# AlexFuster/Neural_network_image_compression

Measured on AMD Instinct MI355X. Metric: Megapixels/sec encode+decode, higher is better.
Workload: dtype fp32 (split-f16x3 MFMA); 1 GPU; config2: 64x256x256x3 u8 synthetic per GPU, encode+decode (torch seed 1000+rank); global_batch=64, parallelism=dp1, weights=seeded spread init (random-init weights of the architecture)

## Files before the change

neural_network_image_compression_amd/csrc/nic_capi.hip:

```cpp

#include <hip/hip_runtime.h>

#include <algorithm>
#include <atomic>
#include <cmath>
#include <condition_variable>
#include <cstdarg>
#include <cstdio>
#include <cstring>
#include <mutex>
#include <string>
#include <thread>
#include <vector>

#include "../../include/nic.h"
#include "nic_kernels.h"

using namespace nic;

namespace {

thread_local std::string g_err;

int fail(int code, const char* fmt, ...) __attribute__((format(printf, 2, 3)));
// ... 511 lines not shown
    const int64_t want[4] = {L->k, L->k, L->transposed ? L->cout : L->cin, L->transposed ? L->cin : L->cout};
    if (ndim != 4 || shape[0] != want[0] || shape[1] != want[1] || shape[2] != want[2] || shape[3] != want[3])
      return fail(NIC_ESHAPE, "nic_set_weights: %s/kernel expects shape (%lld,%lld,%lld,%lld)", lname.c_str(),
                  (long long)want[0], (long long)want[1], (long long)want[2], (long long)want[3]);
    std::vector<float> packed;
    std::vector<uint16_t> packedx;
    const int kexp = repack_kernel(*L, host, packed, packedx);
    HIP_TRY(hipMemcpy(c->wk[L->id] + m * packed.size(), packed.data(), packed.size() * sizeof(float),
                      hipMemcpyHostToDevice));
    if (!packedx.empty()) {
      HIP_TRY(hipMemcpy(c->wx[L->id] + m * packedx.size(), packedx.data(), packedx.size() * sizeof(uint16_t),
                        hipMemcpyHostToDevice));
      c->wscale[L->id][m] = std::ldexp(1.0f, -kexp);
    }
    if (L->id == L_DCONV8) {
      const std::vector<uint16_t> f = proj_fragments(packed, kexp);
      HIP_TRY(hipMemcpy(c->wproj + m * kProjFrag, f.data(), f.size() * sizeof(uint16_t), hipMemcpyHostToDevice));
    }
    c->have_k[model_id][idx] = true;
  } else if (kind == "bias") {
    if (ndim != 1 || shape[0] != L->cout)
      return fail(NIC_ESHAPE, "nic_set_weights: %s/bias expects shape (%d,)", lname.c_str(), L->cout);
    HIP_TRY(hipMemcpy(c->wb[L->id] + m * L->cout, host, L->cout * sizeof(float), hipMemcpyHostToDevice));
    c->have_b[model_id][idx] = true;
  } else {
    return fail(NIC_EINVAL, "nic_set_weights: '%s' is neither kernel nor bias", kind.c_str());
  }
  return NIC_OK;
}

int nic_weights_ready(nic_ctx* c, int* enc, int* dec) {
  if (!c) return fail(NIC_EINVAL, "nic_weights_ready: NULL ctx");
  if (enc) *enc = models_ready(c, 0);
  if (dec) *dec = models_ready(c, 2);
  return NIC_OK;
}

int nic_latent_shape(int h, int w, int* h8, int* w8) {
  if (h <= 0 || w <= 0) return fail(NIC_ESHAPE, "nic_latent_shape: h=%d w=%d must be positive", h, w);
  const SamePad a = same_pad(same_pad(same_pad(h, 5, 2).out, 5, 2).out, 5, 2);
  const SamePad b = same_pad(same_pad(same_pad(w, 5, 2).out, 5, 2).out, 5, 2);
  if (h8) *h8 = a.out;
  if (w8) *w8 = b.out;
  return NIC_OK;
}

int nic_reserve(nic_ctx* c, int n, int h, int w) {
  if (!c) return fail(NIC_EINVAL, "nic_reserve: NULL ctx");
  if (n < 0 || h <= 0 || w <= 0) return fail(NIC_ESHAPE, "nic_reserve: bad shape (%d,%d,%d)", n, h, w);
  DeviceGuard guard(c->device);
  const EncGeom e = enc_geom(n, h, w);
  const DecGeom d = dec_geom(n, e.c8y.out, e.c8x.out);
  float* R[4];
  int rc = ensure_regions(c, std::max(e.r0, d.r0), std::max(e.r123, d.r123), R);
  if (rc) return rc;
  const size_t cb = n > 0 ? hist_scratch_bytes(n, e.c8y.out * e.c8x.out) : 0;
  if (cb > c->counts_bytes) {
    if (c->counts) HIP_TRY(hipFree(c->counts));
    c->counts = nullptr;
    c->counts_bytes = 0;
    HIP_TRY(hipMalloc(&c->counts, cb));
    c->counts_bytes = cb;
  }
  return NIC_OK;
}

}

namespace {

bool use_k3pair() {
  static const bool on = [] {
    const char* e = getenv("NIC_K3P");
    return !(e && e[0] == '0');
  }();
  return on;
}
hipError_t launch_pair(nic_ctx* c, ConvArgs ap, LayerId lb, hipStream_t st) {
  ap.wx2 = c->wx[lb];
  ap.wscale2[0] = c->wscale[lb][0];
  ap.wscale2[1] = c->wscale[lb][1];
  ap.bias2 = c->wb[lb];
  return launch_k3pair_x3(ap, st);
}

bool use_chain() {
  static const bool on = [] {
    const char* e = getenv("NIC_CHAIN");
    return !(e && e[0] == '0');
  }();
  return on;
}

int encode_pass(nic_ctx* c, const uint8_t* rgb, int n, int h, int w, uint8_t* latent, float* prequant,
                hipStream_t st, bool x3, const RangeGuard& rg, bool timed) {
  const EncGeom g = enc_geom(n, h, w);
  float* R[4];
  int rc = ensure_regions(c, g.r0, g.r123, R);
  if (rc) return rc;
  const int P = 3 * n;
  const bool timing_on = c->timing;
  c->timing = timing_on && timed;
  struct Restore {
    nic_ctx* c;
    bool v;
    ~Restore() { c->timing = v; }
  } restore{c, timing_on};

  Conv1Args a1{};
  a1.rg = rg;
  a1.rgb = rgb;
  a1.out = R[0];
  a1.out_s = x3 ? (uint16_t*)R[0] : nullptr;
  a1.w = c->wk[L_CONV1];
  a1.bias = c->wb[L_CONV1];
  a1.P = P;
  a1.nimg = n;
  a1.H = h;
  a1.W = w;
  a1.OH = g.c1y.out;
  a1.OW = g.c1x.out;
  a1.pad_y = g.c1y.lo;
  a1.pad_x = g.c1x.lo;
  Fp32Chain chain{};
  const bool chained = !x3 && rg.gate && use_chain();
  chain.gate = rg;
  chain.q = c->range + 2;
  const bool fuse12 = x3;
  if (!fuse12) TIMED(L_CONV1, chained ? chain_add_conv1(chain, a1) : launch_conv1(a1, st));
  RangeGuard rgl = rg;
  rgl.trips = nullptr;
  auto run = [&](LayerId id, const ConvArgs& a) {
    return chained ? chain_add_layer(chain, id, a) : x3 ? launch_layer_x3(id, a, st) : launch_layer(id, a, st);
  };

  auto conv = [&](LayerId id, const float* in, float* out, const float* res, int H, int W, int OH, int OW, int py,
                  int px) {
    ConvArgs a{};
    a.rg = rgl;
    a.in = in;
    a.out = out;
    a.res = res;
    a.in_s = (const uint16_t*)in;
    a.out_s = (uint16_t*)out;
    a.res_s = (const uint16_t*)res;
    a.zero16 = c->zero16;
    a.w = c->wk[id];
    a.wx = c->wx[id];
    a.wscale[0] = c->wscale[id][0];
    a.wscale[1] = c->wscale[id][1];
    a.bias = c->wb[id];
    a.P = P;
    a.nimg = n;
    a.H = H;
    a.W = W;
    a.OH = OH;
    a.OW = OW;
    a.pad_y = py;
    a.pad_x = px;
    return a;
  };
  const int h1 = g.c1y.out, w1 = g.c1x.out, h2 = g.c2y.out, w2 = g.c2x.out;
  ConvArgs a2 = conv(L_CONV2, R[0], R[1], nullptr, h1, w1, h2, w2, g.c2y.lo, g.c2x.lo);
  if (fuse12) {
    a2.rgb = rgb;
    a2.wx1 = c->wx[L_CONV1];
// ... 12 lines not shown
  if (x3 && use_k3pair() && k3pair_supported(h2, w2)) {
    TIMED(L_CONV4, launch_pair(c, conv(L_CONV3, R[1], R[3], nullptr, h2, w2, h2, w2, 1, 1), L_CONV4, st));
  } else {
    TIMED(L_CONV3, run(L_CONV3, conv(L_CONV3, R[1], R[2], nullptr, h2, w2, h2, w2, 1, 1)));
    TIMED(L_CONV4, run(L_CONV4, conv(L_CONV4, R[2], R[3], R[1], h2, w2, h2, w2, 1, 1)));
  }
  ConvArgs a8 = conv(L_CONV8, R[3], nullptr, nullptr, h2, w2, g.c8y.out, g.c8x.out, g.c8y.lo, g.c8x.lo);
  a8.out_u8 = latent;
  a8.out_f32_latent = prequant;
  if (x3 && c->fold_part) {
    a8.hist_part = c->fold_part;
  }
  TIMED(L_CONV8, run(L_CONV8, a8));
  if (chained) HIP_TRY(launch_fp32_chain(chain, st));
  return NIC_OK;
}

int decode_pass(nic_ctx* c, const uint8_t* latent, int n, int h8, int w8, uint8_t* rgb, float* rgb_f32,
                hipStream_t st, bool x3, const RangeGuard& rg, bool timed) {
  const DecGeom g = dec_geom(n, h8, w8);
  float* R[4];
  int rc = ensure_regions(c, g.r0, g.r123, R);
  if (rc) return rc;
  const int P = 3 * n;
  const bool timing_on = c->timing;
  c->timing = timing_on && timed;
  struct Restore {
    nic_ctx* c;
    bool v;
    ~Restore() { c->timing = v; }
  } restore{c, timing_on};
  RangeGuard rgl = rg;
  rgl.trips = nullptr;
  Fp32Chain chain{};
  const bool chained = !x3 && rg.gate && use_chain();
  chain.gate = rg;
  chain.q = c->range + 2;
  auto run = [&](LayerId id, const ConvArgs& a) {
    return chained ? chain_add_layer(chain, id, a) : x3 ? launch_layer_x3(id, a, st) : launch_layer(id, a, st);
  };
  auto conv = [&](LayerId id, const float* in, float* out, const float* res, int H, int W, int OH, int OW) {
    ConvArgs a{};
    a.rg = rgl;
    a.in = in;
    a.out = out;
    a.res = res;
    a.in_s = (const uint16_t*)in;
    a.out_s = (uint16_t*)out;
    a.res_s = (const uint16_t*)res;
    a.zero16 = c->zero16;
    a.w = c->wk[id];
    a.wx = c->wx[id];
    a.wscale[0] = c->wscale[id][0];
    a.wscale[1] = c->wscale[id][1];
    a.bias = c->wb[id];
    a.P = P;
    a.nimg = n;
    a.H = H;
    a.W = W;
    a.OH = OH;
    a.OW = OW;
    a.pad_y = 1;
    a.pad_x = 1;
    return a;
  };
  ConvArgs d1 = conv(L_DCONV1, nullptr, R[1], nullptr, h8, w8, 2 * h8, 2 * w8);
  d1.in_u8 = latent;
  d1.rg = rg;
  TIMED(L_DCONV1, run(L_DCONV1, d1));
  const int h2 = 2 * h8, w2 = 2 * w8;
  if (x3 && use_k3pair() && k3pair_supported(h2, w2)) {
    TIMED(L_DCONV6, launch_pair(c, conv(L_DCONV5, R[1], R[3], nullptr, h2, w2, h2, w2), L_DCONV6, st));
  } else {
    TIMED(L_DCONV5, run(L_DCONV5, conv(L_DCONV5, R[1], R[2], nullptr, h2, w2, h2, w2)));
    TIMED(L_DCONV6, run(L_DCONV6, conv(L_DCONV6, R[2], R[3], R[1], h2, w2, h2, w2)));
  }
  ConvArgs d7 = conv(L_DCONV7, R[3], R[0], nullptr, h2, w2, 2 * h2, 2 * w2);
  const bool fuse78 = x3;
  if (fuse78) {
    d7.proj = R[0];
    d7.proj_w = c->wproj;
    d7.proj_scale[0] = c->wscale[L_DCONV8][0];
    d7.proj_scale[1] = c->wscale[L_DCONV8][1];
    TIMED(L_DCONV7, launch_dconv7_proj_x3(d7, st));
  } else {
    TIMED(L_DCONV7, run(L_DCONV7, d7));
  }
  Dconv8Args a8{};
  a8.rg = rgl;
  a8.in = R[0];
  a8.in_s = (const uint16_t*)R[0];
  a8.zero16 = c->zero16;
  a8.out_u8 = rgb;
  a8.out_f32 = rgb_f32;
  a8.w = c->wk[L_DCONV8];
  a8.wx = c->wx[L_DCONV8];
  a8.wscale[0] = c->wscale[L_DCONV8][0];
  a8.wscale[1] = c->wscale[L_DCONV8][1];
  a8.bias = c->wb[L_DCONV8];
  a8.nimg = n;
  a8.H = 2 * h2;
  a8.W = 2 * w2;
  if (fuse78) {
    a8.proj = R[0];
    a8.tiles_y7 = (h2 + 7) / 8;
    a8.tiles_x7 = (w2 + 7) / 8;
    TIMED(L_DCONV8, launch_dconv8_gather(a8, st));
  } else {
    TIMED(L_DCONV8, chained ? chain_add_dconv8(chain, a8) : launch_dconv8(a8, st));
  }
  if (chained) HIP_TRY(launch_fp32_chain(chain, st));
  return NIC_OK;
}

bool x3_plane_fits(long long h64, long long w64) { return h64 * w64 * 64 * 4 < (1LL << 30); }

template <class Pass>
int guarded(nic_ctx* c, hipStream_t st, const char* what, bool x3_fits, Pass pass) {
  if (c->precision != NIC_PRECISION_F16X3 || !x3_fits) return pass(false, RangeGuard{}, true);
  if (++c->epoch <= 0) c->epoch = 1;
  RangeGuard prod{};
  prod.flag = c->range;
  prod.epoch = c->epoch;
  int rc = pass(true, prod, true);
  if (rc) return rc;
  if (c->range_policy == NIC_RANGE_FALLBACK) {
    RangeGuard gate{};
    gate.gate = c->range;
    gate.trips = c->range + 1;
    gate.epoch = c->epoch;
    return pass(false, gate, false);
  }
  HIP_TRY(hipMemcpyAsync(c->range_host, c->range, sizeof(int), hipMemcpyDeviceToHost, st));
  HIP_TRY(hipStreamSynchronize(st));
  if (*c->range_host == c->epoch) {
    ++c->error_trips;
    return fail(NIC_ERANGE, "%s: an activation reached the f16 limit of the split-f16 pass (|x| >= 65504); "
                "outputs are undefined (use NIC_RANGE_FALLBACK or NIC_PRECISION_FP32)", what);
  }
  return NIC_OK;
}

void host_chunk_plan(int n, int k, std::vector<int>& lo) {
  k = std::max(1, std::min({k, n, kHostMaxChunks}));
  std::vector<double> wgt(k);
  double tot = 0;
  for (int i = 0; i < k; ++i)
    tot += wgt[i] = (double)(1 << std::min(i, k - 1 - i));
  lo.assign(1, 0);
  double acc = 0;
  for (int i = 0; i < k; ++i) {
    acc += wgt[i];
    const int b = i + 1 == k ? n : std::max(lo.back() + 1, std::min(n - (k - 1 - i), (int)std::lround(n * acc / tot)));
    lo.push_back(b);
  }
}

bool host_pinned(const void* p) {
  hipPointerAttribute_t a{};
  if (hipPointerGetAttributes(&a, p) != hipSuccess) {
    (void)hipGetLastError();
    return false;
  }
  return a.type == hipMemoryTypeHost;
}

int grow_pinned(uint8_t*& p, size_t& have, size_t need) {
// ... 606 lines not shown
```

neural_network_image_compression_amd/csrc/nic_kernels.h:

```cpp
#pragma once
#include <hip/hip_runtime.h>
#include <stdint.h>

namespace nic {

int set_error(int code, const char* msg);

enum InMode { IN_F32 = 0, IN_U8_LATENT = 1, IN_SPLIT = 2, IN_SPLIT_DMA = 3, IN_U8_CODES = 4 };
enum OutMode { OUT_F32 = 0, OUT_U8_LATENT = 1, OUT_SPLIT = 2 };

enum LayerId {
  L_CONV1 = 0, L_CONV2, L_CONV3, L_CONV4, L_CONV8,
  L_DCONV1, L_DCONV5, L_DCONV6, L_DCONV7, L_DCONV8,
  L_COUNT
};

constexpr float kF16Limit = 65504.0f;
struct RangeGuard {
  int* flag = nullptr;
  const int* gate = nullptr;
  int* trips = nullptr;
  int epoch = 0;
};

// ... 15 lines not shown
  const float* bias;
  int P, nimg;
  int H, W;
  int OH, OW;
  int pad_y, pad_x;
  int tiles_x;
  int tiles_y, ntiles;
  int ws_taps;
  int ws_ngrp;
  int ws_blk[9];
  int ws_xcd;
  uint32_t* hist_part;
  const uint16_t* wx2;
  float wscale2[2];
  const float* bias2;
  int seg_rows;
  const uint8_t* rgb;
  const uint16_t* wx1;
  float wscale1[2];
  const float* bias1;
  int H0, W0;
  int p1y, p1x;
  uint16_t* cplane;
  int cp_h, cp_w;
  float* proj;
  const uint16_t* proj_w;
  float proj_scale[2];
};

struct Conv1Args {
  RangeGuard rg;
  const uint8_t* rgb;
  float* out;
  uint16_t* out_s;
  const float* w;
  const float* bias;
  int P, nimg, H, W, OH, OW, pad_y, pad_x, tiles_x, tiles_y;
};

struct Dconv8Args {
  RangeGuard rg;
  const float* in;
  const uint16_t* in_s;
  const char* zero16;
  uint8_t* out_u8;
  float* out_f32;
  const float* w;
  const uint16_t* wx;
  float wscale[2];
  const float* bias;
  int nimg, H, W, tiles_x, tiles_y;
  const float* proj;
  int tiles_y7, tiles_x7;
};

constexpr int kChainMax = 6;
constexpr int kChainQWords = 2 * kChainMax + 1;
struct Fp32Chain {
  RangeGuard gate;
  int* q;
  int nstage;
  int diag_late;
  int total[kChainMax];
  int kind[kChainMax];
  ConvArgs c[kChainMax];
  Conv1Args c1;
  Dconv8Args d8;
};
hipError_t chain_add_layer(Fp32Chain& ch, LayerId id, ConvArgs a);
hipError_t chain_add_conv1(Fp32Chain& ch, Conv1Args a);
hipError_t chain_add_dconv8(Fp32Chain& ch, Dconv8Args a);
hipError_t launch_fp32_chain(const Fp32Chain& ch, hipStream_t st);
void fp32_chain_launch_info(int* blocks_per_cu, int* grid, int* cooperative);

hipError_t upload_constants(const float* u8_to_unit, const float* ycbcr, const float* ycbcr_inv, const float* off);
hipError_t launch_layer(LayerId id, const ConvArgs& a, hipStream_t st);
hipError_t launch_layer_x3(LayerId id, const ConvArgs& a, hipStream_t st);
bool k3pair_supported(int H, int W);
hipError_t launch_k3pair_x3(const ConvArgs& a, hipStream_t st);
hipError_t launch_conv12_x3(const ConvArgs& a, hipStream_t st);
void c12_plane_geom(int OH, int OW, int pad_y, int pad_x, int p1y, int p1x, int* oy, int* ox, int* hp, int* wp);
hipError_t launch_conv1(Conv1Args a, hipStream_t st);
hipError_t launch_dconv8(Dconv8Args a, hipStream_t st);
hipError_t launch_dconv7_proj_x3(const ConvArgs& a, hipStream_t st);
hipError_t launch_dconv8_gather(Dconv8Args a, hipStream_t st);
size_t hist_scratch_bytes(int nimg, int plane_px);
hipError_t launch_hist(const uint8_t* z, int nimg, int plane_px, uint32_t* part, uint32_t* counts, float* bits,
                       hipStream_t st);
bool hist_fold_supported(int nimg, int h8, int w8);
size_t hist_fold_scratch_bytes(int nimg, int h8, int w8);
hipError_t launch_hist_fold(uint32_t* part, const uint8_t* z, int nimg, int h8, int w8, RangeGuard trip,
                            uint32_t* counts, float* bits, hipStream_t st);
hipError_t launch_pack(const uint8_t* src, uint8_t* dst, int nimg, int h8, int w8, bool unpack, hipStream_t st);

constexpr int kSsimScales = 5;

struct SsimScaleArgs {
  const uint8_t* a8;
  const uint8_t* b8;
  const float* af;
  const float* bf;
  double2* part;
  int P, H, W, tiles_x, tiles;
};

struct SsimCombineArgs {
  const double2* part;
  size_t offset[kSsimScales];
  int tiles[kSsimScales];
  int64_t valid[kSsimScales];
  float* out;
  float* per_scale;
};

struct SsimPlan {
  int h[kSsimScales], w[kSsimScales], tiles_x[kSsimScales], tiles[kSsimScales];
  int64_t valid[kSsimScales];
  size_t img_off[kSsimScales];
  size_t part_off[kSsimScales];
  size_t img_bytes, bytes;
};
hipError_t upload_ssim_constants();
void ssim_plan(int nimg, int H, int W, SsimPlan* plan);
hipError_t launch_ms_ssim(const uint8_t* a, const uint8_t* b, int nimg, int H, int W, void* scratch, float* out,
                          float* per_scale, hipStream_t st);
hipError_t launch_sq_err(const uint8_t* a, const uint8_t* b, int nimg, int64_t bytes, unsigned long long* sse,
                         hipStream_t st);

size_t train_scale_work_floats();
size_t train_wgrad_work_floats(int n, int uh, int uw, int kh, int kw, int ca, int cb);
size_t train_gather_work_bytes(int kh, int kw, int cin, int cout);
hipError_t launch_absmax_scale(const float* x, long long n, float* scale, float* work, hipStream_t st);
hipError_t launch_conv_gather(const float* x, int n, int h, int w, int cin, const float* wt, int kh, int kw, int layout,
                              int stride, int pad_y, int pad_x, int transposed, const float* bias, const float* x_scale,
                              const float* w_scale, float* y, int oh, int ow, int cout, int act, void* work, hipStream_t st);
size_t train_abg_work_floats(long long rows, int cols);
hipError_t launch_act_bias_grad(const float* y, const float* dy, long long rows, int cols, int act, float* dz, float* db,
                                float* dz_scale, float* work, hipStream_t st);
hipError_t launch_conv_wgrad(const float* gat, int n, int gh, int gw, int ca, const float* dir, int uh, int uw, int cb,
                             int kh, int kw, int stride, int pad_y, int pad_x, const float* gat_scale,
                             const float* dir_scale, float* dw, float* work, hipStream_t st);
hipError_t launch_adam_keras(const long long* table, int count, long long max_n, float alpha, float beta1,
                             float beta2, float eps, hipStream_t st);
size_t train_ssim_work_floats(int n, long long hw);
hipError_t launch_ssim_map(const float* mx, const float* my, const float* sxy, const float* sxx, int n, long long hw,
                           float c1, float c2, float* out, float* work, hipStream_t st);
hipError_t launch_ssim_map_grad(const float* mx, const float* my, const float* sxy, const float* sxx, const float* g,
                                int n, long long hw, float c1, float c2, float* gmx, float* gmy, float* gsxy,
                                float* gsxx, hipStream_t st);
hipError_t launch_gauss1d(const float* in, int n, int hi, int wi, const float* taps, int nt, int vertical, int adjoint,
                          float* out, int ho, int wo, hipStream_t st);

}
```

neural_network_image_compression_amd/csrc/nic_kernels.hip:

```cpp

#include <hip/hip_runtime.h>
#include <stdint.h>
#include <stdlib.h>
#include <string.h>

#include <algorithm>
#include <type_traits>
#include <utility>

#include "nic_kernels.h"


namespace nic {

static int device_cus();

typedef float f32x2 __attribute__((ext_vector_type(2)));
typedef float f32x4 __attribute__((ext_vector_type(4)));
template <class F, int... I>
__device__ __forceinline__ void static_for_impl(F&& f, std::integer_sequence<int, I...>) {
  (f(std::integral_constant<int, I>{}), ...);
}
template <int N, class F>
__device__ __forceinline__ void static_for(F&& f) {
// ... 1561 lines not shown
#if defined(NIC_DIAG_C12R) && NIC_DIAG_C12R == 3
      if (false)
#endif
      if (i + 1 < ntile) conv1(i + 1);
      C12R_MARK(3);
      dma_wait_all();
      lds_reads_done();
      C12R_MARK(4);
      stage_barrier();
      C12R_MARK(0);
    }
  }
#ifdef NIC_STAMPS
  if (lane == 0) {
    unsigned long long* o = g_stamps + ((size_t)blockIdx.x * 8 + wave) * 8;
#pragma unroll
    for (int q = 0; q < 7; ++q) o[q] = sx[q];
    o[7] = ntile;
    if (wave == 0) {
      g_stamps[256 * 64 + 2 * blockIdx.x] = __builtin_amdgcn_s_memtime() - s_c0;
      g_stamps[256 * 64 + 2 * blockIdx.x + 1] = __builtin_amdgcn_s_memrealtime() - s_rt0;
    }
  }
#endif
#undef C12R_MARK
  range_report(a.rg, rmax);
}

__device__ __forceinline__ int xcd_pos(int b, int nb) {
  const int x = b & 7, q = nb >> 3, r = nb & 7;
  return x * q + (x < r ? x : r) + (b >> 3);
}

__global__ __launch_bounds__(512) void conv12_kernel(ConvArgs a) {
  KT_SCOPE(1);
  using G = GeomS2<32, 8, 8>;
  __shared__ __attribute__((aligned(16)))
  char lds[2 * G::HALO_BYTES + 4 * 4 * 1024 + 4 * C12_PLANE + 16];
  int gi = 0;
  while (gi + 1 < a.ws_ngrp && (int)blockIdx.x >= a.ws_blk[gi + 1]) ++gi;
  const int nb = a.ws_blk[gi + 1] - a.ws_blk[gi];
  const int bi = xcd_pos(blockIdx.x - a.ws_blk[gi], nb);
  if (__builtin_amdgcn_readfirstlane((int)(threadIdx.x >> 6)) < 4)
    c12r_wave<2>(a, lds, gi, bi, nb);
  else
    c12r_wave<1>(a, lds, gi, bi, nb);
}

template <int CIN, int COUT, int NTS, int TH, int OUT_MODE, bool HIST = false>
__global__ __launch_bounds__(64 * (COUT / 16) * NTS) void conv_ws2_kernel(ConvArgs a) {
  KT_SCOPE(3);
  using G = GeomS2<CIN, TH, 8>;
  constexpr int NCG = COUT / 16;
  static_assert(NCG * NTS == 8, "8 waves per block");
  constexpr int PARTS = 2 * (NTS - 1) * NCG * (TH / 2) * 1024;
  __shared__ __attribute__((aligned(16)))
  char lds[2 * G::HALO_BYTES + PARTS + (HIST ? HIST_LDS : 0)];
  int gi = 0;
  while (gi + 1 < a.ws_ngrp && (int)blockIdx.x >= a.ws_blk[gi + 1]) ++gi;
  const int nb = a.ws_blk[gi + 1] - a.ws_blk[gi];
  const int bi = xcd_pos(blockIdx.x - a.ws_blk[gi], nb);
  const int ts = __builtin_amdgcn_readfirstlane((int)(threadIdx.x >> 6)) / NCG;
  static_for<NTS>([&](auto tsc) {
    constexpr int TS = decltype(tsc)::value;
    if (ts == TS) ws2_wave<CIN, COUT, NTS, TH, OUT_MODE, TS, HIST>(a, lds, gi, bi, nb);
  });
}

template <int CIN, int COUT, int TH, int TW, bool RESID, bool TRP, bool PROJ = false>
__global__ __launch_bounds__(64 * (COUT / 16), 2) void conv_ws_kernel(ConvArgs a) {
  KT_SCOPE(6);
  using G = GeomWS<CIN, TH, TW>;
  __shared__ __attribute__((aligned(16)))
  char lds[2 * G::HALO_BYTES + (PROJ ? 2 * (CIN / 32) * 2 * 64 * 16 + TH * TW * COUT * 4 : 0) +
           (RESID && kResDma ? (COUT / 16) * (TH * TW / 16) * 1024 : 0)];
  const int xcd = blockIdx.x & 7, ng = gridDim.x;
  const int lb = a.ws_xcd ? xcd * (ng >> 3) + min(xcd, ng & 7) + (int)(blockIdx.x >> 3) : (int)blockIdx.x;
  int gi = 0;
  while (gi + 1 < a.ws_ngrp && lb >= a.ws_blk[gi + 1]) ++gi;
  const int bi = lb - a.ws_blk[gi], nb = a.ws_blk[gi + 1] - a.ws_blk[gi];
  const int model = gi & 1;
  if constexpr (!TRP) {
    ws_body<CIN, COUT, TH, TW, RESID, 3, 3, false>(a, lds, model, bi, nb, 0, 0, 0);
  } else if (a.ws_ngrp == 2) {
    ws_body<CIN, COUT, TH, TW, false, 3, 3, true, PROJ>(a, lds, model, bi, nb, 16, 1, 1);
    ws_body<CIN, COUT, TH, TW, false, 2, 3, true, PROJ>(a, lds, model, bi, nb, 4, 0, 1, false);
    ws_body<CIN, COUT, TH, TW, false, 3, 2, true, PROJ>(a, lds, model, bi, nb, 10, 1, 0, false);
    ws_body<CIN, COUT, TH, TW, false, 2, 2, true, PROJ>(a, lds, model, bi, nb, 0, 0, 0, false);
  } else {
    switch (gi >> 1) {
      case 0: ws_body<CIN, COUT, TH, TW, false, 2, 2, true, PROJ>(a, lds, model, bi, nb, 0, 0, 0); break;
      case 1: ws_body<CIN, COUT, TH, TW, false, 2, 3, true, PROJ>(a, lds, model, bi, nb, 4, 0, 1); break;
      case 2: ws_body<CIN, COUT, TH, TW, false, 3, 2, true, PROJ>(a, lds, model, bi, nb, 10, 1, 0); break;
      default: ws_body<CIN, COUT, TH, TW, false, 3, 3, true, PROJ>(a, lds, model, bi, nb, 16, 1, 1); break;
    }
  }
}

constexpr int D1_PSB = 64;
constexpr int D1_RPB = 800;
constexpr int D1_HB = 10 * D1_RPB;
constexpr int D1A_LD = 2;
#ifndef NIC_D1A_PF
#define NIC_D1A_PF 2
#endif

template <int KH1, int KW1, int TB1, int PY1, int PX1, int KH2, int KW2, int TB2, int PY2, int PX2>
__device__ __forceinline__ void d1all_wave(const ConvArgs& a, char* lds, int model, int bi, int nb) {
  constexpr int COUT = 64, MT = 4, TAP_BYTES = 32 * COUT * 4, PXB = COUT * 4;
  constexpr int NT1 = KH1 * KW1, NT2 = KH2 * KW2;
  const int wave = __builtin_amdgcn_readfirstlane(threadIdx.x >> 6), cg = wave & 3;
  const int lane = threadIdx.x & 63, g = lane >> 4, l16 = lane & 15;
  const int per_plane = a.tiles_y * a.tiles_x;
  const int p0 = model ? a.nimg : 0, np = model ? a.P - a.nimg : a.nimg;
  const int ntot = np * per_plane;
  const int ntile = bi < ntot ? (ntot - bi + nb - 1) / nb : 0;
  if (ntile == 0) return;

  f16x8 w1[NT1][2], w2[NT2][2];
  float scale;
  f32x4 bias;
  auto load_weights = [&](int m) __attribute__((always_inline)) {
    const char* wsrc = (const char*)a.wx + (size_t)m * 25 * TAP_BYTES;
    auto frag_w = [&](int tap, int hl) {
      return *(const f16x8*)(wsrc + (size_t)tap * TAP_BYTES + ((((g >> 1) * 2 + hl) * 2 + (g & 1)) * COUT + cg * 16 + l16) * 16);
    };
#pragma unroll
    for (int t = 0; t < NT1; ++t)
#pragma unroll
      for (int hl = 0; hl < 2; ++hl) w1[t][hl] = frag_w(TB1 + t, hl);
#pragma unroll
    for (int t = 0; t < NT2; ++t)
#pragma unroll
      for (int hl = 0; hl < 2; ++hl) w2[t][hl] = frag_w(TB2 + t, hl);
    scale = a.wscale[m] * 0.0039215688593685627f;
    bias = *(const f32x4*)(a.bias + m * COUT + cg * 16 + 4 * g);
  };
  load_weights(model);

  int st_lds[D1A_LD], st_hy[D1A_LD], st_hx[D1A_LD];
#pragma unroll
  for (int j = 0; j < D1A_LD; ++j) {
    const int q = threadIdx.x + 512 * j, pix = q >> 3;
    st_hy[j] = q < 800 ? pix / 10 : -1000;
    st_hx[j] = pix - (pix / 10) * 10;
    st_lds[j] = (pix / 10) * D1_RPB + st_hx[j] * D1_PSB + (q & 7) * 8;
  }
  uint32_t cqa[D1A_LD], cqb[D1A_LD];
  TileWalk it_ld, it_run;
  it_ld.init(bi, nb, a.tiles_y, a.tiles_x);
  it_run = it_ld;
  const size_t img_bytes = (size_t)a.H * a.W * 96;
  auto load_codes = [&](uint32_t (&cq)[D1A_LD], bool live) __attribute__((always_inline)) {
    int pl, ty, tx;
    it_ld.take(pl, ty, tx);
    const int p = p0 + pl, type = p / a.nimg;
    const __amdgpu_buffer_rsrc_t rs = __builtin_amdgcn_make_buffer_rsrc(
        (void*)(a.in_u8 + (live ? (size_t)(p % a.nimg) * img_bytes + type * 32 : 0)), (short)0,
        live ? (int)(img_bytes - type * 32) : 0, kBufWord3);
#pragma unroll
    for (int j = 0; j < D1A_LD; ++j) {
      const int gy = ty * 8 - 1 + st_hy[j], gx = tx * 8 - 1 + st_hx[j];
      const bool ok = (unsigned)gy < (unsigned)a.H && (unsigned)gx < (unsigned)a.W;
      cq[j] = __builtin_amdgcn_raw_buffer_load_b32(
          rs, ok ? (unsigned)(((gy * a.W + gx) * 96) + (threadIdx.x & 7) * 4) : kDmaOOR, 0, 0);
    }
  };
  const int st_off = (g & 1) * COUT + cg * 16 + 8 * (g >> 1);
  const unsigned out_plane = (unsigned)((size_t)a.OH * a.OW * PXB);
  unsigned g_off[MT];
#pragma unroll
  for (int m = 0; m < MT; ++m) {
    const int dy = 2 * m + (l16 >> 3), dx = l16 & 7;
    g_off[m] = (unsigned)(((2 * dy) * a.OW + 2 * dx) * PXB + st_off * 2);
  }
  float rmax = 0.f;
  auto phase = [&](const char* buf, const f16x8* wr, auto shape_c, int py, int px, int p, int ty0, int tx0) {
    constexpr int KH = decltype(shape_c)::value / 4, KW = decltype(shape_c)::value % 4, NTAPS = KH * KW;
// ... 26 lines not shown
        acc[m] = __builtin_amdgcn_mfma_f32_16x16x32_f16(wr[2 * t + 1], cur, acc[m], 0, 0, 0);
        acc[m] = __builtin_amdgcn_mfma_f32_16x16x32_f16(wr[2 * t], cur, acc[m], 0, 0, 0);
        if (t + NIC_D1_LA < NTAPS) cur = frag(m, t + NIC_D1_LA);
        __builtin_amdgcn_sched_barrier(0);
      }
    }
    __builtin_amdgcn_s_setprio(0);
    const __amdgpu_buffer_rsrc_t out_rs = __builtin_amdgcn_make_buffer_rsrc(
        (void*)(a.out_s + (size_t)p * out_plane / 2), (short)0, (int)out_plane, kBufWord3);
    const unsigned out_org = (unsigned)(((2 * ty0 + py) * a.OW + 2 * tx0 + px) * PXB);
#pragma unroll
    for (int m = 0; m < MT; ++m) {
      const int y = ty0 + 2 * m + (l16 >> 3), x = tx0 + (l16 & 7);
      f32x4 v;
#pragma unroll
      for (int r = 0; r < 4; ++r) v[r] = leaky02(scale_bias(acc[m][r], scale, bias[r]));
      const bool in = y < a.H && x < a.W;
      if (in) range_track(rmax, v);
      f16x4 hi, lo;
      split4(v, hi, lo);
#ifdef NIC_DIAG_D1NOST
      __builtin_amdgcn_raw_buffer_store_b128(swap16_pair(hi, lo), out_rs, kDmaOOR, 0, 0);
#elif defined(NIC_DIAG_D1LIN)
      {
        const unsigned tq = (unsigned)(((ty0 >> 3) * a.tiles_x + (tx0 >> 3)) * 4 + py * 2 + px) * 4 + cg;
        __builtin_amdgcn_raw_buffer_store_b128(swap16_pair(hi, lo), out_rs, tq * 4096u + (unsigned)(m * 64 + lane) * 16u, 0, 0);
      }
#else
      __builtin_amdgcn_raw_buffer_store_b128(swap16_pair(hi, lo), out_rs, in ? out_org + g_off[m] : kDmaOOR, 0, 0);
#endif
    }
  };
  auto step = [&](int i, uint32_t (&cq)[D1A_LD]) __attribute__((always_inline)) {
    char* buf = lds + (i & 1) * D1_HB;
#pragma unroll
    for (int j = 0; j < D1A_LD; ++j) {
      if (st_hy[j] < 0) continue;
      const uint32_t q = cq[j];
      const f16x4 c = {(_Float16)(float)(q & 255), (_Float16)(float)((q >> 8) & 255),
                       (_Float16)(float)((q >> 16) & 255), (_Float16)(float)(q >> 24)};
      *(f16x4*)(buf + st_lds[j]) = c;
    }
    lds_reads_done();
    stage_barrier();
    int pl, ty, tx;
    it_run.take(pl, ty, tx);
    if constexpr (NIC_D1A_PF == 2) {
      load_codes(cq, i + 2 < ntile);
    } else {
      load_codes(cq, i + 1 < ntile);
    }
    phase(buf, &w1[0][0], std::integral_constant<int, KH1 * 4 + KW1>{}, PY1, PX1, p0 + pl, ty * 8, tx * 8);
    phase(buf, &w2[0][0], std::integral_constant<int, KH2 * 4 + KW2>{}, PY2, PX2, p0 + pl, ty * 8, tx * 8);
  };
  load_codes(cqa, true);
  if constexpr (NIC_D1A_PF == 2) {
    load_codes(cqb, ntile > 1);
    {
      const __amdgpu_buffer_rsrc_t none = __builtin_amdgcn_make_buffer_rsrc((void*)a.out_s, (short)0, 0, kBufWord3);
#pragma unroll
      for (int k = 0; k < 16; ++k) __builtin_amdgcn_raw_buffer_store_b32(0u, none, kDmaOOR + 256u * k, 0, 0);
    }
    int i = 0;
    for (; i + 1 < ntile; i += 2) {
      step(i, cqa);
      step(i + 1, cqb);
    }
    if (i < ntile) step(i, cqa);
  } else {
    for (int i = 0; i < ntile; ++i) step(i, cqa);
  }
  range_report(a.rg, rmax);
}

__global__ __launch_bounds__(512, 1) void dconv1_all_kernel(ConvArgs a) {
  KT_SCOPE(5);
  __shared__ __attribute__((aligned(16))) char lds[2 * D1_HB];
  const int gi = (int)blockIdx.x >= a.ws_blk[1] ? 1 : 0;
  const int bi = blockIdx.x - a.ws_blk[gi], nb = a.ws_blk[gi + 1] - a.ws_blk[gi];
  if (threadIdx.x < 256)
    d1all_wave<3, 3, 16, 1, 1, 2, 2, 0, 0, 0>(a, lds, gi, bi, nb);
  else
    d1all_wave<2, 3, 4, 0, 1, 3, 2, 10, 1, 0>(a, lds, gi, bi, nb);
}

constexpr int K3P_MAX_W = 64;
constexpr int K3P_SW = 62;
constexpr int K3P_REC = 256;
constexpr int K3P_RW = K3P_MAX_W + 4;
constexpr int K3P_ROWB = K3P_RW * K3P_REC;
constexpr int K3P_NI = 5, K3P_NC = 4;
#ifndef NIC_K3P_DMAB
#define NIC_K3P_DMAB 1
#endif
constexpr bool kK3pDmaB = NIC_K3P_DMAB != 0;
constexpr int K3P_LDS = (K3P_NI + K3P_NC) * K3P_ROWB;

__device__ __forceinline__ int k3p_off(int rec, int chunk) { return rec * K3P_REC + ((chunk ^ ((2 * rec) & 15)) << 4); }

constexpr int K3P_MAX_GRID = 320;
struct K3Ranges {
  int start[K3P_MAX_GRID + 1];
};
template <int MT, bool SKEW, bool STRIP>
__global__ __launch_bounds__(512, 1) void conv_k3pair_kernel(ConvArgs a, K3Ranges rng) {
  KT_SCOPE(2);
  constexpr int COUT = 64, KST = 2;
  __shared__ __attribute__((aligned(16))) char lds[K3P_LDS];
  char* in_ring = lds;
  char* c3_ring = lds + K3P_NI * K3P_ROWB;
  const int wave = __builtin_amdgcn_readfirstlane(threadIdx.x >> 6);
  const int role = wave >> 2, w = wave & 3;
  const int lane = threadIdx.x & 63, g = lane >> 4, l16 = lane & 15;
  const int H = a.H, W = a.W;
  static_assert(!STRIP || MT == 4, "strips are 4 M tiles wide");
  const int nstrips = STRIP ? a.tiles_x : 1;
  const long long total_rows = (long long)a.P * nstrips * H;
  long long g0, g1;
  if (rng.start[0] >= 0) {
    g0 = rng.start[blockIdx.x];
    g1 = rng.start[blockIdx.x + 1];
  } else {
    const long long per_block = (total_rows + gridDim.x - 1) / gridDim.x;
    g0 = (long long)blockIdx.x * per_block;
    g1 = min(g0 + per_block, total_rows);
  }
  const unsigned plane_bytes = (unsigned)(H * W) * K3P_REC;

  for (int q = threadIdx.x; q < (K3P_NI + K3P_NC) * K3P_RW * 16; q += 512) {
    const int row = q / (K3P_RW * 16), r = q - row * (K3P_RW * 16), rec = r >> 4;
    if (rec == 0 || rec > W) *(u32x4*)(lds + row * K3P_ROWB + r * 16) = (u32x4){0u, 0u, 0u, 0u};
  }

  int bx[3];
#pragma unroll
  for (int kw = 0; kw < 3; ++kw) bx[kw] = k3p_off(l16 + kw, g);
  const int chunk_st = (g & 1) * 8 + 2 * w + (g >> 1);
  const int chunk_rh = 2 * w + (g >> 1), rsub = 8 * (g & 1);

  f16x8 wr[9][KST][2];
  int model = -1;
  float scale = 0.f;
  f32x4 bias = {};
  float rmax = 0.f;
  auto load_weights = [&](int m) {
    const uint16_t* wx = role == 0 ? a.wx : a.wx2;
    constexpr int TAP_BYTES = 64 * COUT * 4;
    const char* wsrc = (const char*)wx + (size_t)m * 9 * TAP_BYTES;
#pragma unroll
    for (int t = 0; t < 9; ++t)
#pragma unroll
      for (int ks = 0; ks < KST; ++ks)
#pragma unroll
        for (int hl = 0; hl < 2; ++hl)
          wr[t][ks][hl] = *(const f16x8*)(wsrc + (size_t)t * TAP_BYTES +
                                          ((((2 * ks + (g >> 1)) * 2 + hl) * 2 + (g & 1)) * COUT + w * 16 + l16) * 16);
    scale = role == 0 ? a.wscale[m] : a.wscale2[m];
    bias = *(const f32x4*)((role == 0 ? a.bias : a.bias2) + m * COUT + 16 * w + 4 * g);
  };

  constexpr int ca_off = STRIP ? 0 : 1, rb_off = STRIP ? 2 : 1, jmax = STRIP ? K3P_SW : 64;
  constexpr int rec0 = STRIP ? 0 : 1;
  int sx0 = 0;
  auto dma_row = [&](const __amdgpu_buffer_rsrc_t& rs, int y, int slot) {
    const int npiece = STRIP ? K3P_RW / 4 : (W * 16 + 63) / 64;
    const int xi0 = STRIP ? sx0 - 2 : -1;
// ... 1016 lines not shown
  a.tiles_y = (a.OH + TH - 1) / TH;
  a.tiles_x = (a.OW + 7) / 8;
  const long long per_plane = (long long)a.tiles_y * a.tiles_x;
  const long long nt = per_plane * a.P;
  if (nt == 0) return hipSuccess;
  if (nt > INT32_MAX || a.P != 3 * a.nimg) return hipErrorInvalidValue;
  a.ntiles = (int)nt;
  a.ws_taps = 25;
  a.ws_ngrp = 2;
  int by, bc;
  ws2_groups(a.nimg, per_plane, &by, &bc);
  a.ws_blk[0] = 0;
  a.ws_blk[1] = by;
  a.ws_blk[2] = by + bc;
  if constexpr (PIPE12) {
    hipLaunchKernelGGL(conv12_kernel, dim3(a.ws_blk[2]), dim3(512), 0, st, a);
  } else if constexpr (OUT_MODE == OUT_U8_LATENT) {
    if (a.hist_part) {
      if (!hist_fold_supported(a.nimg, a.OH, a.OW)) return hipErrorInvalidValue;
      hipLaunchKernelGGL((conv_ws2_kernel<CIN, COUT, NTS, TH, OUT_MODE, true>), dim3(a.ws_blk[2]), dim3(512), 0, st, a);
    } else {
      hipLaunchKernelGGL((conv_ws2_kernel<CIN, COUT, NTS, TH, OUT_MODE>), dim3(a.ws_blk[2]), dim3(512), 0, st, a);
    }
  } else {
    hipLaunchKernelGGL((conv_ws2_kernel<CIN, COUT, NTS, TH, OUT_MODE>), dim3(a.ws_blk[2]), dim3(512), 0, st, a);
  }
  return hipGetLastError();
}

hipError_t launch_conv12_x3(const ConvArgs& a0, hipStream_t st) {
  ConvArgs a = a0;
  if (!a.rgb || !a.wx1 || !a.bias1 || a.H0 <= 0 || a.W0 <= 0) return hipErrorInvalidValue;
  if (!a.cplane || a.OH <= 0 || a.OW <= 0) return hipErrorInvalidValue;
  int oy, ox;
  c12_plane_geom(a.OH, a.OW, a.pad_y, a.pad_x, a.p1y, a.p1x, &oy, &ox, &a.cp_h, &a.cp_w);
  if ((long long)a.cp_h * a.cp_w * 2 >= (1LL << 31)) return hipErrorInvalidValue;
  const long long per_img = (long long)a.cp_h * (a.cp_w / 4);
  if (per_img == 0 || a.nimg == 0) return hipSuccess;
  if (a.nimg > 65535 || (long long)a.W0 * 3 >= (1LL << 31)) return hipErrorInvalidValue;
  hipLaunchKernelGGL(colour_split_kernel, dim3((unsigned)((per_img + 255) / 256), a.nimg),
                     dim3(256), 0, st, a.rgb, a.cplane, a.nimg, a.H0, a.W0, oy, ox, a.cp_h, a.cp_w);
  hipError_t e = hipGetLastError();
  if (e != hipSuccess) return e;
  return launch_ws2<32, 64, 2, 8, OUT_SPLIT, true>(a, st);
}

static hipError_t launch_dconv1_all(ConvArgs a, hipStream_t st) {
  a.tiles_y = (a.H + 7) / 8;
  a.tiles_x = (a.W + 7) / 8;
  const long long per_plane = (long long)a.tiles_y * a.tiles_x, nt = per_plane * a.P;
  if (nt == 0) return hipSuccess;
  if (nt > INT32_MAX || a.P != 3 * a.nimg || a.OH != 2 * a.H || a.OW != 2 * a.W || !a.in_u8) return hipErrorInvalidValue;
  if ((long long)a.OH * a.OW * 256 >= (1LL << 31)) return hipErrorInvalidValue;
  const long long target = device_cus();
  const long long ty = (long long)a.nimg * per_plane, tc = 2LL * a.nimg * per_plane;
  const int by = (int)std::max(1LL, std::min(ty, (target + 1) / 3)), bc = (int)std::max(1LL, std::min(tc, target - by));
  a.ws_ngrp = 2;
  a.ws_blk[0] = 0;
  a.ws_blk[1] = by;
  a.ws_blk[2] = by + bc;
  hipLaunchKernelGGL(dconv1_all_kernel, dim3(a.ws_blk[2]), dim3(512), 0, st, a);
  return hipGetLastError();
}

hipError_t launch_layer_x3(LayerId id, const ConvArgs& a, hipStream_t st) {
  switch (id) {
    case L_CONV2:
      return launch_ws2<32, 64, 2, 8, OUT_SPLIT>(a, st);
    case L_CONV3:
    case L_DCONV5:
      return launch_ws<64, 64, 8, 8, false, false>(a, st);
    case L_CONV4:
    case L_DCONV6:
      return launch_ws<64, 64, 8, 8, true, false>(a, st);
    case L_CONV8:
      return launch_ws2<64, 32, 4, 4, OUT_U8_LATENT>(a, st);
    case L_DCONV1:
      return launch_dconv1_all(a, st);
    default:
      return hipErrorInvalidValue;
  }
}

hipError_t launch_dconv7_proj_x3(const ConvArgs& a, hipStream_t st) {
  if (!a.proj || !a.proj_w || a.OH != 2 * a.H || a.OW != 2 * a.W) return hipErrorInvalidValue;
  return launch_ws<64, 64, 8, 8, false, true, true>(a, st);
}

hipError_t launch_conv1(Conv1Args a, hipStream_t st) {
  a.tiles_y = (a.OH + C1_T - 1) / C1_T;
  a.tiles_x = (a.OW + C1_T - 1) / C1_T;
  const long long jobs = (long long)a.tiles_y * a.tiles_x * a.P;
  if (jobs == 0) return hipSuccess;
  if (jobs > INT32_MAX) return hipErrorInvalidValue;
  hipLaunchKernelGGL(conv1_colour_kernel, dim3(fp32_grid(a.rg, jobs)), dim3(256), 0,
                     st, a);
  return hipGetLastError();
}

hipError_t launch_dconv8(Dconv8Args a, hipStream_t st) {
  a.tiles_y = (a.H + D8_TH - 1) / D8_TH;
  a.tiles_x = (a.W + D8_TW - 1) / D8_TW;
  const long long jobs = (long long)a.tiles_y * a.tiles_x * a.nimg;
  if (jobs == 0) return hipSuccess;
  if (jobs > INT32_MAX) return hipErrorInvalidValue;
  hipLaunchKernelGGL(dconv8_colour_kernel, dim3(fp32_grid(a.rg, jobs)), dim3(256), 0,
                     st, a);
  return hipGetLastError();
}

hipError_t launch_dconv8_gather(Dconv8Args a, hipStream_t st) {
  if (!a.proj || (a.H & 1) || (a.W & 1)) return hipErrorInvalidValue;
  if (a.tiles_y7 != (a.H / 2 + 7) / 8 || a.tiles_x7 != (a.W / 2 + 7) / 8) return hipErrorInvalidValue;
  const int tiles_y = (a.H + 15) / 16;
  a.tiles_x = (a.W + 15) / 16;
  hipLaunchKernelGGL(dconv8_gather_kernel, dim3(tiles_y * a.tiles_x, a.nimg), dim3(256), 0, st, a);
  return hipGetLastError();
}

int hist_chunks(int nimg, int plane_px, int* chunk_vec, int blocks) {
  const long long nvec = (long long)plane_px * 6;
  long long cv = ((nvec * nimg + blocks - 1) / blocks + 255) / 256 * 256;
  cv = cv < 256 ? 256 : (cv > 16384 ? 16384 : cv);
  *chunk_vec = (int)cv;
  return (int)((nvec + cv - 1) / cv);
}

size_t hist_scratch_bytes(int nimg, int plane_px) {
  int cv;
  return (size_t)3 * nimg * hist_chunks(nimg, plane_px, &cv, 1536) * 256 * sizeof(uint32_t);
}

hipError_t launch_hist(const uint8_t* z, int nimg, int plane_px, uint32_t* part, uint32_t* counts, float* bits,
                       hipStream_t st) {
  const char* hv = getenv("NIC_HIST");
  const int force = !hv ? 0 : hv[0] == 'b' ? 1 : hv[0] == 's' ? 2 : 0;
  const long long total = (long long)plane_px * 96 * nimg;
  const bool big = force ? force == 1 : total >= (24ll << 20);
  int chunk_vec;
  const int chunks = hist_chunks(nimg, plane_px, &chunk_vec, big ? 512 : 1536);
  if (big)
    hipLaunchKernelGGL((latent_hist_kernel<16, false, 1024>), dim3(chunks, nimg), dim3(1024), 0, st, z, nimg, plane_px, part,
                       chunk_vec);
  else
    hipLaunchKernelGGL((latent_hist_kernel<8, false, 256>), dim3(chunks, nimg), dim3(256), 0, st, z, nimg, plane_px, part,
                       chunk_vec);
  hipError_t e = hipGetLastError();
  if (e != hipSuccess) return e;
  hipLaunchKernelGGL(hist_entropy_kernel, dim3(3 * nimg), dim3(1024), 0, st, part, chunks, (float)plane_px * 32.0f,
                     counts, bits);
  return hipGetLastError();
}

hipError_t launch_hist_fold(uint32_t* part, const uint8_t* z, int nimg, int h8, int w8, RangeGuard trip,
                            uint32_t* counts, float* bits, hipStream_t st) {
  if (!hist_fold_supported(nimg, h8, w8)) return hipErrorInvalidValue;
  hipLaunchKernelGGL(hist_fold_kernel, dim3(3 * nimg), dim3(256), 0, st, part, nimg, z, h8 * w8, trip,
                     (float)h8 * w8 * 32.0f, counts, bits);
  return hipGetLastError();
}

hipError_t launch_pack(const uint8_t* z, uint8_t* out, int nimg, int h8, int w8, bool unpack, hipStream_t st) {
  const size_t plane_elems = (size_t)h8 * w8 * 32;
  const size_t total = plane_elems * nimg;
  const int blocks = (int)((total + 255) / 256 < 8192 ? (total + 255) / 256 : 8192);
  if (unpack)
    hipLaunchKernelGGL(unpack_latent_kernel, dim3(blocks), dim3(256), 0, st, z, out, plane_elems, nimg);
  else
// ... 6 lines not shown
```

Before: 3184 MP/s.

## Add opt-in all-phase dconv7 kernel with in-block projection pipelining

Adds a new dconv7 transposed-conv kernel that computes all four sub-pixel phases per tile in one block. Waves are split into two roles with weights held in registers and LDS, and the dconv8 projection is overlapped through LDS flag handshakes. It is gated behind NIC_D7=1, which defaults to off. The existing ws kernel also drops its per-phase grid-split path and always loops over all four phases when the transposed path is used, which changes how the default path behaves.

New measurement: 3188 MP/s, median of 6. No clear change (+0.1%).

```diff
diff --git a/neural_network_image_compression_amd/csrc/nic_capi.hip b/neural_network_image_compression_amd/csrc/nic_capi.hip
--- a/neural_network_image_compression_amd/csrc/nic_capi.hip
+++ b/neural_network_image_compression_amd/csrc/nic_capi.hip
@@ -617,6 +617,14 @@
   ap.wscale2[1] = c->wscale[lb][1];
   ap.bias2 = c->wb[lb];
   return launch_k3pair_x3(ap, st);
+}
+
+bool use_d7all() {
+  static const bool on = [] {
+    const char* e = getenv("NIC_D7");
+    return e && e[0] == '1';
+  }();
+  return on;
 }
 
 bool use_chain() {
@@ -795,7 +803,7 @@
     d7.proj_w = c->wproj;
     d7.proj_scale[0] = c->wscale[L_DCONV8][0];
     d7.proj_scale[1] = c->wscale[L_DCONV8][1];
-    TIMED(L_DCONV7, launch_dconv7_proj_x3(d7, st));
+    TIMED(L_DCONV7, launch_dconv7_proj_x3(d7, st, use_d7all()));
   } else {
     TIMED(L_DCONV7, run(L_DCONV7, d7));
   }
diff --git a/neural_network_image_compression_amd/csrc/nic_kernels.h b/neural_network_image_compression_amd/csrc/nic_kernels.h
--- a/neural_network_image_compression_amd/csrc/nic_kernels.h
+++ b/neural_network_image_compression_amd/csrc/nic_kernels.h
@@ -121,7 +121,7 @@
 void c12_plane_geom(int OH, int OW, int pad_y, int pad_x, int p1y, int p1x, int* oy, int* ox, int* hp, int* wp);
 hipError_t launch_conv1(Conv1Args a, hipStream_t st);
 hipError_t launch_dconv8(Dconv8Args a, hipStream_t st);
-hipError_t launch_dconv7_proj_x3(const ConvArgs& a, hipStream_t st);
+hipError_t launch_dconv7_proj_x3(const ConvArgs& a, hipStream_t st, bool all_phases = false);
 hipError_t launch_dconv8_gather(Dconv8Args a, hipStream_t st);
 size_t hist_scratch_bytes(int nimg, int plane_px);
 hipError_t launch_hist(const uint8_t* z, int nimg, int plane_px, uint32_t* part, uint32_t* counts, float* bits,
diff --git a/neural_network_image_compression_amd/csrc/nic_kernels.hip b/neural_network_image_compression_amd/csrc/nic_kernels.hip
--- a/neural_network_image_compression_amd/csrc/nic_kernels.hip
+++ b/neural_network_image_compression_amd/csrc/nic_kernels.hip
@@ -1667,18 +1667,11 @@
   const int model = gi & 1;
   if constexpr (!TRP) {
     ws_body<CIN, COUT, TH, TW, RESID, 3, 3, false>(a, lds, model, bi, nb, 0, 0, 0);
-  } else if (a.ws_ngrp == 2) {
+  } else {
     ws_body<CIN, COUT, TH, TW, false, 3, 3, true, PROJ>(a, lds, model, bi, nb, 16, 1, 1);
     ws_body<CIN, COUT, TH, TW, false, 2, 3, true, PROJ>(a, lds, model, bi, nb, 4, 0, 1, false);
     ws_body<CIN, COUT, TH, TW, false, 3, 2, true, PROJ>(a, lds, model, bi, nb, 10, 1, 0, false);
     ws_body<CIN, COUT, TH, TW, false, 2, 2, true, PROJ>(a, lds, model, bi, nb, 0, 0, 0, false);
-  } else {
-    switch (gi >> 1) {
-      case 0: ws_body<CIN, COUT, TH, TW, false, 2, 2, true, PROJ>(a, lds, model, bi, nb, 0, 0, 0); break;
-      case 1: ws_body<CIN, COUT, TH, TW, false, 2, 3, true, PROJ>(a, lds, model, bi, nb, 4, 0, 1); break;
-      case 2: ws_body<CIN, COUT, TH, TW, false, 3, 2, true, PROJ>(a, lds, model, bi, nb, 10, 1, 0); break;
-      default: ws_body<CIN, COUT, TH, TW, false, 3, 3, true, PROJ>(a, lds, model, bi, nb, 16, 1, 1); break;
-    }
   }
 }
 
@@ -1871,6 +1864,253 @@
     d1all_wave<3, 3, 16, 1, 1, 2, 2, 0, 0, 0>(a, lds, gi, bi, nb);
   else
     d1all_wave<2, 3, 4, 0, 1, 3, 2, 10, 1, 0>(a, lds, gi, bi, nb);
+}
+
+constexpr int D7A_LA = 5, D7A_LB = 3;
+constexpr int D7A_HALO = GeomWS<64, 8, 8>::HALO_BYTES;
+constexpr int D7A_W8 = 2 * D7A_HALO;
+constexpr int D7A_HPROJ = D7A_W8 + 2 * 2 * 2 * 64 * 16;
+constexpr int D7A_WLO = D7A_HPROJ + 2 * 64 * 256;
+constexpr int D7A_FLAG = D7A_WLO + (D7A_LA + D7A_LB) * 8192;
+constexpr int D7A_LDS = D7A_FLAG + 32;
+static_assert(D7A_LDS <= 160 * 1024, "one block per CU");
+
+template <int KH_, int KW_, int TB_, int PY_, int PX_, int U0_>
+struct D7Phase {
+  static constexpr int KH = KH_, KW = KW_, TB = TB_, PY = PY_, PX = PX_, U0 = U0_, NTAPS = KH_ * KW_;
+};
+
+template <int ROLE>
+__device__ __forceinline__ void d7all_wave(const ConvArgs& a, char* lds, int model, int bi, int nb) {
+  constexpr int CIN = 64, COUT = 64, TH = 8, TW = 8, KST = 2, MT = 4, MC = 2, TAP_BYTES = CIN * COUT * 4;
+  using G = GeomWS<CIN, TH, TW>;
+  static_assert(MT % MC == 0, "whole chunks of pixel tiles");
+  using HP = HaloDma<G, CIN, 8>;
+  using P1 = std::conditional_t<ROLE == 0, D7Phase<3, 3, 16, 1, 1, 0>, D7Phase<2, 3, 4, 0, 1, 0>>;
+  using P2 = std::conditional_t<ROLE == 0, D7Phase<2, 2, 0, 0, 0, 9>, D7Phase<3, 2, 10, 1, 0, 6>>;
+  constexpr int NT = P1::NTAPS + P2::NTAPS, NL = ROLE == 0 ? D7A_LA : D7A_LB, NR = NT - NL;
+  typedef const __attribute__((address_space(3))) f16x8* lds_frag_t;
+
+  const int wave = __builtin_amdgcn_readfirstlane(threadIdx.x >> 6), wq = wave & 3;
+  const int lane = threadIdx.x & 63, g = lane >> 4, l16 = lane & 15;
+  const int co0 = wq * 16 + 4 * g;
+  const int per_plane = a.tiles_y * a.tiles_x;
+  const int p0 = model ? a.nimg : 0, np = model ? a.P - a.nimg : a.nimg;
+  const int ntot = np * per_plane;
+  const int ntile = bi < ntot ? (ntot - bi + nb - 1) / nb : 0;
+  if (ntile == 0) return;
+
+  f16x8 wh[NT][KST], wl[NR][KST];
+  const unsigned wl_lds = lds_off(lds + D7A_WLO + (ROLE * 4 * D7A_LA + wq * NL) * 2048 + lane * 16);
+  {
+    const char* wsrc = (const char*)a.wx + (size_t)model * 25 * TAP_BYTES;
+    static_for<NT>([&](auto uc) {
+      constexpr int u = decltype(uc)::value;
+      constexpr int tap = u < P1::NTAPS ? P1::TB + u : P2::TB + (u - P1::NTAPS);
+#pragma unroll
+      for (int ks = 0; ks < KST; ++ks)
+#pragma unroll
+        for (int hl = 0; hl < 2; ++hl) {
+          const f16x8 f = *(const f16x8*)(wsrc + (size_t)tap * TAP_BYTES +
+                                          ((((2 * ks + (g >> 1)) * 2 + hl) * 2 + (g & 1)) * COUT + wq * 16 + l16) * 16);
+          if (hl == 0)
+            wh[u][ks] = f;
+          else if constexpr (u < NR)
+            wl[u][ks] = f;
+          else
+            *(f16x8*)(lds + D7A_WLO + (ROLE * 4 * D7A_LA + wq * NL) * 2048 + ((u - NR) * 2 + ks) * 1024 + lane * 16) = f;
+        }
+    });
+  }
+  const float scale = a.wscale[model];
+  const f32x4 bias = *(const f32x4*)(a.bias + model * COUT + co0);
+  constexpr int W8F = 2 * KST * 2;
+  const f16x8* w8lds = (const f16x8*)(lds + D7A_W8) + lane;
+  const float scale8 = a.proj_scale[model];
+  char* hproj = lds + D7A_HPROJ + ROLE * (64 * 256);
+  {
+    const f16x8* src = (const f16x8*)a.proj_w + (size_t)model * W8F * 64;
+    for (int q = threadIdx.x; q < W8F * 64; q += 512) ((f16x8*)(lds + D7A_W8))[q] = src[q];
+  }
+  int* rflag = (int*)(lds + D7A_FLAG) + ROLE * 4;
+  if (lane == 0) rflag[wq] = 0;
+  auto reads_published = [&](int gen) {
+    lds_reads_done();
+    asm volatile("" ::: "memory");
+    __hip_atomic_store(rflag + wq, gen, __ATOMIC_RELAXED, __HIP_MEMORY_SCOPE_WORKGROUP);
+  };
+  auto reads_wait = [&](int gen) {
+#pragma unroll
+    for (int k = 0; k < 4; ++k)
+      while (__hip_atomic_load(rflag + k, __ATOMIC_RELAXED, __HIP_MEMORY_SCOPE_WORKGROUP) < gen)
+        __builtin_amdgcn_s_sleep(1);
+    asm volatile("" ::: "memory");
+  };
+
+  int bx[3];
+#pragma unroll
+  for (int kw = 0; kw < 3; ++kw) {
+    const int hx = (l16 & 7) + kw;
+    bx[kw] = (l16 >> 3) * G::RPB + hx * G::PSB + (G::chunk_at(g, hx) << 4);
+  }
+  HP hp;
+  const unsigned plane_bytes = (unsigned)((size_t)a.H * a.W * CIN * 4);
+  hp.init(wave, lane, a.W);
+  TileWalk it_issue, it_ep;
+  it_issue.init(bi, nb, a.tiles_y, a.tiles_x);
+  it_ep = it_issue;
+  auto issue = [&](int i) {
+    int pl, ty, tx;
+    it_issue.take(pl, ty, tx);
+    hp.issue(lds + (i & 1) * G::HALO_BYTES, (const char*)a.in_s + (size_t)(p0 + pl) * plane_bytes, plane_bytes, a.W,
+             ty * TH - a.pad_y, tx * TW - a.pad_x, wave);
+  };
+
+  f32x4 acc[MC];
+  f16x8 fb[MC][2];
+  int ep_p = 0, ep_y = 0, ep_x = 0;
+  float rmax = 0.f;
+  auto stream = [&](auto ph, const char* buf, int m0) {
+    using PH = decltype(ph);
+    constexpr int KW = PH::KW, NSTEP = PH::NTAPS * KST;
+    unsigned bb[KW];
+#pragma unroll
+    for (int kw = 0; kw < KW; ++kw) bb[kw] = lds_off(buf) + bx[kw];
+    auto frag = [&](int m, int st, int hl) {
+      const int t = st / KST, ks = st - t * KST, kh = t / KW, kw = t - kh * KW;
+      return *(lds_frag_t)(lds_at(bb[kw] ^ ((2 * hl + ks) << 6)) + (2 * (m0 + m) + kh) * G::RPB);
+    };
+    auto wlo_lds = [&](int st) {
+      return *(lds_frag_t)lds_at(wl_lds + (unsigned)((PH::U0 * KST + st - NR * KST) * 1024));
+    };
+#pragma unroll
+    for (int m = 0; m < MC; ++m) {
+      acc[m] = (f32x4){0.f, 0.f, 0.f, 0.f};
+      fb[m][0] = frag(m, 0, 0);
+      fb[m][1] = frag(m, 0, 1);
+    }
+    f16x8 wls[2];
+    if constexpr (PH::U0 >= NR) wls[0] = wlo_lds(0);
+    __builtin_amdgcn_s_setprio(1);
+    static_for<NSTEP>([&](auto sc) {
+      constexpr int st = decltype(sc)::value, u = PH::U0 + st / KST, ks = st % KST;
+      if constexpr (st + 1 < NSTEP && PH::U0 + (st + 1) / KST >= NR) wls[(st + 1) & 1] = wlo_lds(st + 1);
+      f16x8 wlo;
+      if constexpr (u >= NR)
+        wlo = wls[st & 1];
+      else
+        wlo = wl[u][ks];
+#pragma unroll
+      for (int m = 0; m < MC; ++m) {
+        acc[m] = __builtin_amdgcn_mfma_f32_16x16x32_f16(wlo, fb[m][0], acc[m], 0, 0, 0);
+        acc[m] = __builtin_amdgcn_mfma_f32_16x16x32_f16(wh[u][ks], fb[m][1], acc[m], 0, 0, 0);
+        acc[m] = __builtin_amdgcn_mfma_f32_16x16x32_f16(wh[u][ks], fb[m][0], acc[m], 0, 0, 0);
+        if (st + 1 < NSTEP) {
+          fb[m][0] = frag(m, st + 1, 0);
+          fb[m][1] = frag(m, st + 1, 1);
+        }
+        __builtin_amdgcn_sched_barrier(0);
+      }
+    });
+    __builtin_amdgcn_s_setprio(0);
+  };
+  auto park = [&](int m0) {
+#pragma unroll
+    for (int mm = 0; mm < MC; ++mm) {
+      const int m = m0 + mm;
+      const int y = ep_y + 2 * m + (l16 >> 3), x = ep_x + (l16 & 7);
+      f32x4 v;
+#pragma unroll
+      for (int r = 0; r < 4; ++r) v[r] = leaky02(scale_bias(acc[mm][r], scale, bias[r]));
+      if (y < a.H && x < a.W) range_track(rmax, v);
+      f16x4 hi, lo;
+      split4(v, hi, lo);
+      const u32x4 q = swap16_pair(hi, lo);
+      const int pp = 16 * m + l16, ch = (g & 1) * 8 + 2 * wq + (g >> 1);
+      *(u32x4*)(hproj + pp * 256 + ((ch ^ (pp & 15)) << 4)) = q;
+    }
+  };
+  const int ppx = 16 * wq + l16;
+  auto project = [&](int py, int px) {
+    f32x4 pd[2] = {(f32x4){0.f, 0.f, 0.f, 0.f}, (f32x4){0.f, 0.f, 0.f, 0.f}};
+    f16x8 pah, pal, pwh, pwl;
+    auto load_a = [&](int ks) {
+      pah = *(const f16x8*)(hproj + ppx * 256 + (((4 * ks + g) ^ (ppx & 15)) << 4));
+      pal = *(const f16x8*)(hproj + ppx * 256 + (((8 + 4 * ks + g) ^ (ppx & 15)) << 4));
+    };
+    auto load_w = [&](int j) {
+      pwh = w8lds[(((j & 1) * KST + (j >> 1)) * 2 + 0) * 64];
+      pwl = w8lds[(((j & 1) * KST + (j >> 1)) * 2 + 1) * 64];
+    };
+    load_a(0);
+    load_w(0);
+#pragma unroll
+    for (int j = 0; j < 4; ++j) {
+      f32x4& d = pd[j & 1];
+      d = __builtin_amdgcn_mfma_f32_16x16x32_f16(pal, pwh, d, 0, 0, 0);
+      d = __builtin_amdgcn_mfma_f32_16x16x32_f16(pah, pwl, d, 0, 0, 0);
+      d = __builtin_amdgcn_mfma_f32_16x16x32_f16(pah, pwh, d, 0, 0, 0);
+      if (j == 1) load_a(1);
+      if (j + 1 < 4) load_w(j + 1);
+    }
+    float* dst = a.proj +
+                 ((((size_t)ep_p * 4 + 2 * py + px) * a.tiles_y + ep_y / TH) * a.tiles_x + ep_x / TW) * (25 * 64) +
+                 16 * wq + 4 * g;
+#pragma unroll
+    for (int nt = 0; nt < 2; ++nt) {
+      const int tap = 16 * nt + l16;
+      if (tap < 25) *(f32x4*)(dst + tap * 64) = pd[nt] * scale8;
+    }
+  };
+
+  issue(0);
+  for (int i = 0; i <= ntile; ++i) {
+    dma_wait_all();
+    lds_reads_done();
+    stage_barrier();
+    if (i + 1 < ntile) issue(i + 1);
+    if (i > 0) {
+      project(P2::PY, P2::PX);
+      reads_published(2 * i);
+    }
+    if (i == ntile) break;
+    {
+      int pl, ty, tx;
+      it_ep.take(pl, ty, tx);
+      ep_p = p0 + pl;
+      ep_y = ty * TH;
+      ep_x = tx * TW;
+    }
+    const char* buf = lds + (i & 1) * G::HALO_BYTES;
+    stream(P1{}, buf, 0);
+    if (i > 0) reads_wait(2 * i);
+    park(0);
+    stream(P1{}, buf, MC);
+    park(MC);
+    lds_reads_done();
+    stage_barrier();
+    project(P1::PY, P1::PX);
+    reads_published(2 * i + 1);
+    stream(P2{}, buf, 0);
+    reads_wait(2 * i + 1);
+    park(0);
+    stream(P2{}, buf, MC);
+    park(MC);
+  }
+  range_report(a.rg, rmax);
+}
+
+__global__ __launch_bounds__(512, 1) void dconv7_all_kernel(ConvArgs a) {
+  KT_SCOPE(6);
+  __shared__ __attribute__((aligned(16))) char lds[D7A_LDS];
+  const int xcd = blockIdx.x & 7, ng = gridDim.x;
+  const int lb = xcd * (ng >> 3) + min(xcd, ng & 7) + (int)(blockIdx.x >> 3);
+  const int gi = lb >= a.ws_blk[1] ? 1 : 0;
+  const int bi = lb - a.ws_blk[gi], nb = a.ws_blk[gi + 1] - a.ws_blk[gi];
+  if (threadIdx.x < 256)
+    d7all_wave<0>(a, lds, gi, bi, nb);
+  else
+    d7all_wave<1>(a, lds, gi, bi, nb);
 }
 
 constexpr int K3P_MAX_W = 64;
@@ -3053,8 +3293,30 @@
   }
 }
 
-hipError_t launch_dconv7_proj_x3(const ConvArgs& a, hipStream_t st) {
+static hipError_t launch_dconv7_all(ConvArgs a, hipStream_t st) {
+  a.tiles_y = (a.H + 7) / 8;
+  a.tiles_x = (a.W + 7) / 8;
+  const long long per_plane = (long long)a.tiles_y * a.tiles_x, nt = per_plane * a.P;
+  if (nt == 0) return hipSuccess;
+  if (nt > INT32_MAX || a.P != 3 * a.nimg) return hipErrorInvalidValue;
+  if ((long long)a.H * a.W * 64 * 4 >= (1LL << 30)) return hipErrorInvalidValue;
+  a.ntiles = (int)nt;
+  a.ws_taps = 25;
+  const long long target = device_cus();
+  const long long ty = (long long)a.nimg * per_plane, tc = 2LL * a.nimg * per_plane;
+  const int by = (int)std::max(1LL, std::min(ty, (target + 1) / 3)), bc = (int)std::max(1LL, std::min(tc, target - by));
+  a.ws_ngrp = 2;
+  a.ws_blk[0] = 0;
+  a.ws_blk[1] = by;
+  a.ws_blk[2] = by + bc;
+  a.ws_xcd = 1;
+  hipLaunchKernelGGL(dconv7_all_kernel, dim3(a.ws_blk[2]), dim3(512), 0, st, a);
+  return hipGetLastError();
+}
+
+hipError_t launch_dconv7_proj_x3(const ConvArgs& a, hipStream_t st, bool all_phases) {
   if (!a.proj || !a.proj_w || a.OH != 2 * a.H || a.OW != 2 * a.W) return hipErrorInvalidValue;
+  if (all_phases) return launch_dconv7_all(a, st);
   return launch_ws<64, 64, 8, 8, false, true, true>(a, st);
 }
 
```
